# hongfz16/Garment4D

Hardware: AMD Instinct MI355X
Metric: point-cloud frames/s (FPS+ball_query+SA-MLP+LBS), B=8 N=8192 (higher is better)
Workload: dtype f32

## Files before the change

garment4d_amd/csrc/api.hip:

```cpp
#include <stdarg.h>
#include <stddef.h>
#include <stdlib.h>
#include <string.h>

#include "mlp_common.h"

namespace g4d {
static thread_local char g_err[512] = "";

void set_error(const char *fmt, ...) {
    va_list ap;
    va_start(ap, fmt);
    vsnprintf(g_err, sizeof(g_err), fmt, ap);
    va_end(ap);
}

static int g_contract = -1;

static int parse_contract(const char *e) {
    if (!e || !*e) return G4D_CONTRACT_NVCC;
    if (!strcmp(e, "0") || !strcmp(e, "off") || !strcmp(e, "none")) return G4D_CONTRACT_OFF;
    if (!strcmp(e, "2") || !strcmp(e, "chain") || !strcmp(e, "inner")) return G4D_CONTRACT_CHAIN;
    return G4D_CONTRACT_NVCC;
}

static thread_local int t_contract = -1;

int distance_contraction() {
    if (t_contract >= 0) return t_contract;
    int m = __atomic_load_n(&g_contract, __ATOMIC_RELAXED);
    if (m < 0) {
        m = parse_contract(getenv("G4D_DIST_CONTRACT"));
        __atomic_store_n(&g_contract, m, __ATOMIC_RELAXED);
    }
    return m;
}
}

namespace g4d {
namespace {
struct Tune { const char *key; long long value; int state; };
Tune g_tune[] = {{"sa_table_persistent", 0, 0}, {"sa_table_min_rows", 0, 0}, {"sa_table_128", 0, 0}, {"sa_table_oversub", 0, 0}, {"sa_table_dedup", 0, 0}, {"fp_table_persistent", 0, 0},
                 {"fp_table_min_rows", 0, 0}, {"gemm_tile", 0, 0}, {"gemm_tile_min_rows", 0, 0}, {"gemm_tile_min_cout", 0, 0}, {"gemm_tile_min_kpad", 0, 0}, {"fp_init_persistent", 0, 0}, {"fp_init_min_rows", 0, 0},
                 {"fp_head_bf16_persistent", 0, 0}, {"fp_head_bf16_min_rows", 0, 0}, {"sa_group_bf16_persistent", 0, 0}, {"sa_group_bf16_min_rows", 0, 0}};
}
struct ThreadTune { long long value; bool set; };
thread_local ThreadTune t_tune[sizeof(g_tune) / sizeof(g_tune[0])] = {};

long long tuning(const char *key, long long dflt) {
    int i = 0;
    for (Tune &t : g_tune) {
        const int slot = i++;
        if (strcmp(t.key, key)) continue;
        if (t_tune[slot].set) return t_tune[slot].value;
        int st = __atomic_load_n(&t.state, __ATOMIC_ACQUIRE);
        if (st == 0) {
            char env[64] = "G4D_";
            size_t n = 4;
            for (const char *c = key; *c && n + 1 < sizeof(env); ++c) env[n++] = (char)((*c >= 'a' && *c <= 'z') ? *c - 32 : *c);
            env[n] = 0;
            const char *e = getenv(env);
            const long long v = e && *e ? atoll(e) : dflt;
            int expect = 0;
            if (__atomic_compare_exchange_n(&t.state, &expect, 3, false, __ATOMIC_ACQ_REL, __ATOMIC_ACQUIRE)) {
                __atomic_store_n(&t.value, v, __ATOMIC_RELAXED);
                expect = 3;
                __atomic_compare_exchange_n(&t.state, &expect, 1, false, __ATOMIC_ACQ_REL, __ATOMIC_ACQUIRE);
                return v;
            }
            st = expect;
            if (st == 3) return v;
        }
        return __atomic_load_n(&t.value, __ATOMIC_RELAXED);
    }
    return dflt;
}
}

extern "C" int g4d_tuning_set(const char *key, long long value) {
    if (key)
        for (g4d::Tune &t : g4d::g_tune)
            if (!strcmp(t.key, key)) {
                __atomic_store_n(&t.value, value, __ATOMIC_RELAXED);
                __atomic_store_n(&t.state, 2, __ATOMIC_RELEASE);
                return G4D_OK;
            }
    g4d::set_error("g4d_tuning_set: unknown key '%s'", key ? key : "(null)");
    return G4D_EINVAL;
}

extern "C" int g4d_tuning_set_thread(const char *key, long long value, int set) {
    if (key) {
        int i = 0;
        for (g4d::Tune &t : g4d::g_tune) {
            const int slot = i++;
            if (!strcmp(t.key, key)) {
                g4d::t_tune[slot].value = value;
                g4d::t_tune[slot].set = set != 0;
                return G4D_OK;
            }
        }
    }
    g4d::set_error("g4d_tuning_set_thread: unknown key '%s'", key ? key : "(null)");
    return G4D_EINVAL;
}

extern "C" int g4d_version(void) { return 263;  }
extern "C" const char *g4d_last_error(void) { return g4d::g_err; }

extern "C" int g4d_get_distance_contraction(void) { return g4d::distance_contraction(); }
extern "C" int g4d_set_distance_contraction_thread(int mode) {
    const int prev = g4d::t_contract;
    if (mode < -1 || mode > G4D_CONTRACT_CHAIN) {
        g4d::set_error("g4d_set_distance_contraction_thread: mode %d is not -1 (no override) or one of G4D_CONTRACT_OFF/NVCC/CHAIN", mode);
        return -2;
    }
    g4d::t_contract = mode;
    return prev;
}

extern "C" int g4d_set_distance_contraction(int mode) {
    const int saved = g4d::t_contract;
    g4d::t_contract = -1;
    const int prev = g4d::distance_contraction();
    g4d::t_contract = saved;
    if (mode < G4D_CONTRACT_OFF || mode > G4D_CONTRACT_CHAIN) {
        g4d::set_error("g4d_set_distance_contraction: mode %d is not one of G4D_CONTRACT_OFF/NVCC/CHAIN", mode);
        return -1;
    }
    __atomic_store_n(&g4d::g_contract, mode, __ATOMIC_RELAXED);
    return prev;
}

namespace g4d {
struct CopySegs { float *dst[4]; const float *src[4]; long long n[4]; long long first_block[5]; };
__global__ void __launch_bounds__(256) copy_segments_kernel(const CopySegs c, int nseg) {
    int s = 0;
    while (s + 1 < nseg && (long long)blockIdx.x >= c.first_block[s + 1]) ++s;
    const long long i0 = ((long long)blockIdx.x - c.first_block[s]) * 1024 + threadIdx.x * 4;
    float *d = c.dst[s];
    const float *p = c.src[s];
    const long long n = c.n[s];
    if (i0 + 3 < n && ((reinterpret_cast<size_t>(d) | reinterpret_cast<size_t>(p)) & 15) == 0) {
        *reinterpret_cast<float4 *>(d + i0) = *reinterpret_cast<const float4 *>(p + i0);
    } else {
        for (int e = 0; e < 4; ++e)
            if (i0 + e < n) d[i0 + e] = p[i0 + e];
    }
}
}

extern "C" int g4d_copy_segments_f32(int nseg, float *const *dst, const float *const *src, const long long *nfloats, g4d_stream_t stream) {
    G4D_REQUIRE(nseg >= 0 && nseg <= 4 && (nseg == 0 || (dst && src && nfloats)), "g4d_copy_segments_f32: 0..4 segments");
    g4d::CopySegs c = {};
    long long blocks = 0;
    int k = 0;
    for (int i = 0; i < nseg; ++i) {
        G4D_REQUIRE(nfloats[i] >= 0 && (nfloats[i] == 0 || (dst[i] && src[i])), "g4d_copy_segments_f32: bad segment %d", i);
        if (nfloats[i] == 0) continue;
        c.dst[k] = dst[i]; c.src[k] = src[i]; c.n[k] = nfloats[i]; c.first_block[k] = blocks;
        blocks += (nfloats[i] + 1023) / 1024;
        ++k;
    }
    if (k == 0) return G4D_OK;
    c.first_block[k] = blocks;
    G4D_REQUIRE(blocks < (1ll << 31), "g4d_copy_segments_f32: too large");
    hipLaunchKernelGGL(g4d::copy_segments_kernel, dim3((unsigned)blocks), dim3(256), 0, reinterpret_cast<hipStream_t>(stream), c, k);
    return g4d::check_launch("g4d_copy_segments_f32");
}

namespace g4d {
static StackCall stack_call(const char *name, const g4d_mlp_args &a) {
    StackCall c = {};
    c.name = name; c.mode = a.mode; c.rows = a.rows;
    LinearArgs &in = c.in;
    in.K = a.K0; in.out = a.out; in.ldo = a.ldo; in.col0 = a.col0; in.pool = a.pool; in.S = a.S;
    in.X = a.X; in.ldx = a.ldx;
    in.xyz = a.xyz; in.new_xyz = a.new_xyz; in.feats = a.feats; in.idx = a.idx; in.N = a.N; in.P = a.P; in.C = a.C; in.use_xyz = a.use_xyz;
    in.known_feats = a.known_feats; in.skip = a.skip; in.dist2 = a.dist2; in.nn_idx = a.nn_idx; in.C2 = a.C2; in.C1 = a.C1; in.m = a.m; in.n = a.n;
    in.rowptr = a.rowptr; in.colidx = a.colidx; in.vals = a.vals; in.Vg = a.Vg;
    c.nlayers = a.nlayers; c.W = a.W; c.scale = a.scale; c.shift = a.shift; c.Kpad = a.Kpad; c.Cout = a.Cout; c.relu = a.relu;
    c.tap_layer = a.tap_layer; c.tap_out = a.tap_out; c.tap_ld = a.tap_ld; c.unknown_grid = a.unknown_grid;
    return c;
}

int stack_call_check(const StackCall &c, const StackRules &r) {
    const int S = c.in.S, pool = c.in.pool;
    G4D_REQUIRE(c.mode >= 0 && c.mode <= (r.csr ? LOAD_CSR : LOAD_INTERP), "%s: %s", c.name, r.bad_mode);
    if (r.max_layers) G4D_REQUIRE(c.nlayers >= 1 && c.nlayers <= r.max_layers, "%s: 1..%d layers", c.name, r.max_layers);
    G4D_REQUIRE(c.rows >= 0 && c.rows < r.max_rows && c.in.K > 0, "%s: bad sizes", c.name);
    if (c.rows == 0) return kEmptyLaunch;
    G4D_REQUIRE(has_layer_arrays(c), "%s: null pointer", c.name);
    if (!r.max_layers) G4D_REQUIRE(g4d_mlp_chain_supported(c.nlayers, c.Cout), "%s: unsupported layer widths (see g4d_mlp_chain_supported)", c.name);
    G4D_REQUIRE(pool >= 0 && pool <= 2, "%s: pool must be 0|1|2", c.name);
    if (pool) G4D_REQUIRE((S == 4 || S == 8 || S == 16 || S == 32 || S == 64) && c.rows % S == 0, "%s: pooling needs S in {4,8,16,32,64}", c.name);
    for (int l = 0; l < c.nlayers; ++l) {
        const void *const *Wl = c.W + (size_t)l * r.w_pieces;
        G4D_REQUIRE(Wl[0] && (r.w_pieces == 1 || (Wl[1] && Wl[2])) && c.scale[l] && c.shift[l] && c.Kpad[l] % r.kpad_multiple == 0 && c.Cout[l] > 0, "%s: bad layer %d", c.name, l);
    }
    G4D_REQUIRE(tap_layer_of(c) < c.nlayers - 1, "%s: tap must be a hidden layer", c.name);
    return G4D_OK;
}
}

extern "C" unsigned g4d_mlp_args_size(void) { return (unsigned)sizeof(g4d_mlp_args); }

extern "C" int g4d_mlp_run(int family, const g4d_mlp_args *args, g4d_stream_t stream) {
    using namespace g4d;
    G4D_REQUIRE(args, "g4d_mlp_run: null argument block");
    G4D_REQUIRE(args->version == G4D_MLP_ARGS_VERSION, "g4d_mlp_run: argument block version %u, this library speaks %d", args->version, G4D_MLP_ARGS_VERSION);
    G4D_REQUIRE(args->size >= 16 && args->size <= sizeof(g4d_mlp_args), "g4d_mlp_run: argument block of %u bytes, this library's is %u (a newer caller?)",
                args->size, (unsigned)sizeof(g4d_mlp_args));
    g4d_mlp_args a;
    memset(&a, 0, sizeof(a));
    memcpy(&a, args, args->size);
    if (args->size < offsetof(g4d_mlp_args, tap_layer) + sizeof(int)) a.tap_layer = -1;
    if (family != G4D_MLP_CHAIN_BF16) a.unknown_grid = nullptr;
    hipStream_t st = reinterpret_cast<hipStream_t>(stream);
    switch (family) {
        case G4D_MLP_STACK_F32: return mlp_stack_f32_run(stack_call("g4d_mlp_stack_f32", a), st);
        case G4D_MLP_STACK_BF16: return mlp_stack_bf16_run(stack_call("g4d_mlp_stack_bf16", a), st);
        case G4D_MLP_WAVE_F32: return mlp_wave_f32_run(stack_call("g4d_mlp_wave_f32", a), st);
        case G4D_MLP_CHAIN_F32: return mlp_chain_f32_run(stack_call("g4d_mlp_chain_f32", a), st);
        case G4D_MLP_CHAIN_BF16: return mlp_chain_bf16_run(stack_call("g4d_mlp_chain_bf16", a), st);
        case G4D_MLP_CHAIN_BF16X3: return mlp_chain_bf16x3_run(stack_call("g4d_mlp_chain_bf16x3", a), st);
    }
    set_error("g4d_mlp_run: unknown kernel family %d", family);
    return G4D_EINVAL;
}

#define G4D_MLP_LOADERS                                                                                                                       \
    int mode, long long rows, int K0,  const float *X, int ldx,                                                            \
     int N, int P, int S, int C, int use_xyz, const float *xyz, const float *new_xyz, const float *feats, const int *idx,        \
     int n, int m, int C2, int C1, const float *known_feats, const float *skip, const float *dist2, const int *nn_idx
#define G4D_MLP_LAYERS(WT)                                                                                                                    \
    int nlayers, const WT *const *W, const float *const *scale, const float *const *shift, const int *Kpad, const int *Cout, const int *relu, \
     int pool, float *out, int ldo, int col0
#define G4D_MLP_COMMON                                                                                                                        \
    mode, rows, K0, X, ldx, N, P, S, C, use_xyz, xyz, new_xyz, feats, idx, n, m, C2, C1, known_feats, skip, dist2, nn_idx, nlayers,         \
    reinterpret_cast<const void *const *>(W), scale, shift, Kpad, Cout, relu, pool, out, ldo, col0

static g4d_mlp_args pack_args(G4D_MLP_LOADERS, G4D_MLP_LAYERS(void), int tap_layer = -1, float *tap_out = nullptr, int tap_ld = 0) {
    g4d_mlp_args a;
    memset(&a, 0, sizeof(a));
    a.size = (unsigned)sizeof(a); a.version = G4D_MLP_ARGS_VERSION;
    a.mode = mode; a.rows = rows; a.K0 = K0; a.X = X; a.ldx = ldx;
    a.N = N; a.P = P; a.S = S; a.C = C; a.use_xyz = use_xyz; a.xyz = xyz; a.new_xyz = new_xyz; a.feats = feats; a.idx = idx;
    a.n = n; a.m = m; a.C2 = C2; a.C1 = C1; a.known_feats = known_feats; a.skip = skip; a.dist2 = dist2; a.nn_idx = nn_idx;
    a.nlayers = nlayers; a.W = W; a.scale = scale; a.shift = shift; a.Kpad = Kpad; a.Cout = Cout; a.relu = relu;
    a.pool = pool; a.out = out; a.ldo = ldo; a.col0 = col0; a.tap_layer = tap_layer; a.tap_out = tap_out; a.tap_ld = tap_ld;
    return a;
}

extern "C" int g4d_mlp_stack_f32(G4D_MLP_LOADERS,  int Vg, const int *rowptr, const int *colidx, const float *vals, G4D_MLP_LAYERS(float),
                                 int tap_layer, float *tap_out, int tap_ld, g4d_stream_t stream) {
    g4d_mlp_args a = pack_args(G4D_MLP_COMMON, tap_layer, tap_out, tap_ld);
    a.Vg = Vg; a.rowptr = rowptr; a.colidx = colidx; a.vals = vals;
    return g4d_mlp_run(G4D_MLP_STACK_F32, &a, stream);
}

extern "C" int g4d_mlp_stack_bf16(G4D_MLP_LOADERS,  int Vg, const int *rowptr, const int *colidx, const float *vals, G4D_MLP_LAYERS(unsigned short),
                                  int tap_layer, float *tap_out, int tap_ld, g4d_stream_t stream) {
    g4d_mlp_args a = pack_args(G4D_MLP_COMMON, tap_layer, tap_out, tap_ld);
    a.Vg = Vg; a.rowptr = rowptr; a.colidx = colidx; a.vals = vals;
    return g4d_mlp_run(G4D_MLP_STACK_BF16, &a, stream);
}

extern "C" int g4d_mlp_wave_f32(G4D_MLP_LOADERS,  int Vg, const int *rowptr, const int *colidx, const float *vals, G4D_MLP_LAYERS(float),
                                g4d_stream_t stream) {
    g4d_mlp_args a = pack_args(G4D_MLP_COMMON);
    a.Vg = Vg; a.rowptr = rowptr; a.colidx = colidx; a.vals = vals;
    return g4d_mlp_run(G4D_MLP_WAVE_F32, &a, stream);
}

extern "C" int g4d_mlp_chain_f32(G4D_MLP_LOADERS, G4D_MLP_LAYERS(float), int tap_layer, float *tap_out, int tap_ld, g4d_stream_t stream) {
    g4d_mlp_args a = pack_args(G4D_MLP_COMMON, tap_layer, tap_out, tap_ld);
    return g4d_mlp_run(G4D_MLP_CHAIN_F32, &a, stream);
}

extern "C" int g4d_mlp_chain_bf16(G4D_MLP_LOADERS, G4D_MLP_LAYERS(unsigned short), int tap_layer, float *tap_out, int tap_ld, g4d_stream_t stream) {
    g4d_mlp_args a = pack_args(G4D_MLP_COMMON, tap_layer, tap_out, tap_ld);
    return g4d_mlp_run(G4D_MLP_CHAIN_BF16, &a, stream);
}

extern "C" int g4d_mlp_chain_cells_bf16(G4D_MLP_LOADERS, G4D_MLP_LAYERS(unsigned short), int tap_layer, float *tap_out, int tap_ld, const void *unknown_grid,
                                        g4d_stream_t stream) {
    g4d_mlp_args a = pack_args(G4D_MLP_COMMON, tap_layer, tap_out, tap_ld);
    a.unknown_grid = unknown_grid;
    return g4d_mlp_run(G4D_MLP_CHAIN_BF16, &a, stream);
}

extern "C" int g4d_mlp_chain_bf16x3(G4D_MLP_LOADERS, G4D_MLP_LAYERS(unsigned short), int tap_layer, float *tap_out, int tap_ld, g4d_stream_t stream) {
    g4d_mlp_args a = pack_args(G4D_MLP_COMMON, tap_layer, tap_out, tap_ld);
    return g4d_mlp_run(G4D_MLP_CHAIN_BF16X3, &a, stream);
}
```

garment4d_amd/csrc/fp_table.hip:

```cpp
#include <cstdlib>

#include "mlp_common.h"

namespace g4d {

typedef float f32x4u __attribute__((ext_vector_type(4), aligned(4)));

struct FpTabArgs {
    int rows, n, m;
    const float *tab;
    const float *dist2;
    const int *nn_idx;
    const unsigned char *perm_rec;
    size_t perm_stride;
    const float *ps, *pf;
    const float *W2, *sc2, *sh2, *W3, *sc3, *sh3, *W4, *sc4, *sh4;
    int cout4, relu4;
    float *out;  int ldo;
    float *tap;  int tap_ld;
};

constexpr int kC1 = 128, kC2 = 64, kC3 = 32, kC4 = 16;
constexpr int kT1 = kC1 / 16, kT2 = kC2 / 16, kT3 = kC3 / 16;
template <bool PERM, int kD, bool HEAD = true>
__global__ void __launch_bounds__(256, kD <= 4 ? 3 : 2) fp_table_head_kernel(const FpTabArgs a) {
    static_assert(kT1 % kD == 0, "ring depth divides the k-steps of a tile");
    constexpr int NW2 = kC1 * kC2, NW3 = kC2 * kC3, NW4 = kC3 * kC4;
    __shared__ __attribute__((aligned(16))) float s_w2[NW2], s_w3[NW3], s_w4[NW4];
    __shared__ __attribute__((aligned(16))) float s_ps[kC1], s_pf[kC1], s_sc2[kC2], s_sh2[kC2], s_sc3[kC3], s_sh3[kC3], s_sc4[kC4], s_sh4[kC4];
    const int tid = threadIdx.x;
    for (int i = tid; i < NW2 / 4; i += 256) reinterpret_cast<f32x4 *>(s_w2)[i] = reinterpret_cast<const f32x4 *>(a.W2)[i];
    if constexpr (HEAD) {
        for (int i = tid; i < NW3 / 4; i += 256) reinterpret_cast<f32x4 *>(s_w3)[i] = reinterpret_cast<const f32x4 *>(a.W3)[i];
        for (int i = tid; i < NW4 / 4; i += 256) reinterpret_cast<f32x4 *>(s_w4)[i] = reinterpret_cast<const f32x4 *>(a.W4)[i];
    }
    if (tid < kC1) { s_ps[tid] = a.ps[tid]; s_pf[tid] = a.pf[tid]; }
    if (tid < kC2) { s_sc2[tid] = a.sc2[tid]; s_sh2[tid] = a.sh2[tid]; }
    if constexpr (HEAD) {
        if (tid < kC3) { s_sc3[tid] = a.sc3[tid]; s_sh3[tid] = a.sh3[tid]; }
        if (tid < kC4) { s_sc4[tid] = a.sc4[tid]; s_sh4[tid] = a.sh4[tid]; }
    }
    __syncthreads();

    const int lane = tid & 63, wave = __builtin_amdgcn_readfirstlane(tid >> 6);
    const int fi = lane & 15, fq = lane >> 4;
    const int ntile = (a.rows + 15) >> 4;
    const int nwaves = gridDim.x * 4, wg = blockIdx.x * 4 + wave;
    if (wg >= ntile) return;
    const int iters = (ntile - wg + nwaves - 1) / nwaves;
    auto tile_of = [&](int it) { return min(wg + it * nwaves, ntile - 1); };

    struct Raw { int i0, i1, i2; float d0, d1, d2; int orow; };
    auto load_raw = [&](int tile) {
        Raw r;
        const int row = min(tile * 16 + fi, a.rows - 1);
        const int *ix = a.nn_idx + (size_t)row * 3;
        const float *dd = a.dist2 + (size_t)row * 3;
        r.i0 = ix[0]; r.i1 = ix[1]; r.i2 = ix[2];
        r.d0 = dd[0]; r.d1 = dd[1]; r.d2 = dd[2];
        const int b0 = __builtin_amdgcn_readfirstlane((tile * 16) / a.n);
        const int b = b0 + (row >= (b0 + 1) * a.n ? 1 : 0);
        r.orow = row;
        if constexpr (PERM) r.orow = b * a.n + reinterpret_cast<const int *>(a.perm_rec + (size_t)b * a.perm_stride)[4 * (row - b * a.n) + 3];
        return r;
    };
    struct Ctx { float w0, w1, w2; unsigned k0, k1, k2; int orow; };
    auto make = [&](int tile, const Raw &r) {
        Ctx c;
        const float r0 = 1.0f / (__fsqrt_rn(r.d0) + 1e-8f), r1 = 1.0f / (__fsqrt_rn(r.d1) + 1e-8f), r2 = 1.0f / (__fsqrt_rn(r.d2) + 1e-8f);
        const float norm = (r0 + r1) + r2;
        c.w0 = r0 / norm; c.w1 = r1 / norm; c.w2 = r2 / norm;
        const int row = min(tile * 16 + fi, a.rows - 1);
        const int b0 = __builtin_amdgcn_readfirstlane((tile * 16) / a.n);
        const unsigned base = (unsigned)(b0 + (row >= (b0 + 1) * a.n ? 1 : 0)) * (unsigned)a.m;
        c.k0 = (base + (unsigned)r.i0) * kC1 + fq * 4; c.k1 = (base + (unsigned)r.i1) * kC1 + fq * 4; c.k2 = (base + (unsigned)r.i2) * kC1 + fq * 4;
        c.orow = r.orow;
        return c;
    };
    struct Item { f32x4 t0, t1, t2; };
    auto load_item = [&](const Ctx &c, int ks) {
        Item x;
        x.t0 = *reinterpret_cast<const f32x4u *>(a.tab + c.k0 + ks * 16);
        x.t1 = *reinterpret_cast<const f32x4u *>(a.tab + c.k1 + ks * 16);
        x.t2 = *reinterpret_cast<const f32x4u *>(a.tab + c.k2 + ks * 16);
        return x;
    };

    Raw rawn = load_raw(tile_of(0));
    Ctx cur = make(tile_of(0), rawn);
    rawn = load_raw(tile_of(1));
    Item ring[kD];
#pragma unroll
    for (int d = 0; d < kD; ++d) ring[d] = load_item(cur, d);
    for (int it = 0; it < iters; ++it) {
        const int tile = tile_of(it);
        const Ctx nxt = make(tile_of(it + 1), rawn);
        rawn = load_raw(tile_of(it + 2));
        f32x4 h2[kT2];
#pragma unroll
        for (int ct = 0; ct < kT2; ++ct) h2[ct] = (f32x4){0.f, 0.f, 0.f, 0.f};
#pragma unroll
        for (int ks = 0; ks < kT1; ++ks) {
            __builtin_amdgcn_sched_barrier(0);
            const Item x = ring[ks % kD];
            ring[ks % kD] = ks + kD < kT1 ? load_item(cur, ks + kD) : load_item(nxt, ks + kD - kT1);
            const int k0 = ks * 16 + fq * 4;
            const f32x4 ps = *reinterpret_cast<const f32x4 *>(s_ps + k0), pf = *reinterpret_cast<const f32x4 *>(s_pf + k0);
            f32x4 h1;
#pragma unroll
            for (int e = 0; e < 4; ++e) {
                const float v = cur.w0 * x.t0[e] + cur.w1 * x.t1[e] + cur.w2 * x.t2[e];
                h1[e] = fmaxf(__builtin_fmaf(v, ps[e], pf[e]), 0.f);
            }
#pragma unroll
            for (int ct = 0; ct < kT2; ++ct) {
                const f32x4 w = *reinterpret_cast<const f32x4 *>(s_w2 + ((ct * kT1 + ks) * 64 + lane) * 4);
#pragma unroll
                for (int e = 0; e < 4; ++e) h2[ct] = __builtin_amdgcn_mfma_f32_16x16x4f32(w[e], h1[e], h2[ct], 0, 0, 0);
            }
        }
        __builtin_amdgcn_sched_barrier(0);
        const bool row_ok = tile * 16 + fi < a.rows;
#pragma unroll
        for (int ct = 0; ct < kT2; ++ct) {
            const f32x4 sc = *reinterpret_cast<const f32x4 *>(s_sc2 + ct * 16 + fq * 4), sh = *reinterpret_cast<const f32x4 *>(s_sh2 + ct * 16 + fq * 4);
#pragma unroll
            for (int r = 0; r < 4; ++r) h2[ct][r] = fmaxf(__builtin_fmaf(h2[ct][r], sc[r], sh[r]), 0.f);
            if (row_ok) *reinterpret_cast<f32x4 *>(a.tap + (size_t)cur.orow * a.tap_ld + ct * 16 + fq * 4) = h2[ct];
        }
        if constexpr (HEAD) {
        __builtin_amdgcn_sched_barrier(0);
        f32x4 h3[kT3];
#pragma unroll
        for (int ct = 0; ct < kT3; ++ct) h3[ct] = (f32x4){0.f, 0.f, 0.f, 0.f};
#pragma unroll
        for (int ks = 0; ks < kT2; ++ks) {
            __builtin_amdgcn_sched_barrier(0);
#pragma unroll
            for (int ct = 0; ct < kT3; ++ct) {
                const f32x4 w = *reinterpret_cast<const f32x4 *>(s_w3 + ((ct * kT2 + ks) * 64 + lane) * 4);
#pragma unroll
                for (int e = 0; e < 4; ++e) h3[ct] = __builtin_amdgcn_mfma_f32_16x16x4f32(w[e], h2[ks][e], h3[ct], 0, 0, 0);
            }
        }
        __builtin_amdgcn_sched_barrier(0);
#pragma unroll
        for (int ct = 0; ct < kT3; ++ct) {
            const f32x4 sc = *reinterpret_cast<const f32x4 *>(s_sc3 + ct * 16 + fq * 4), sh = *reinterpret_cast<const f32x4 *>(s_sh3 + ct * 16 + fq * 4);
#pragma unroll
            for (int r = 0; r < 4; ++r) h3[ct][r] = fmaxf(__builtin_fmaf(h3[ct][r], sc[r], sh[r]), 0.f);
        }
        __builtin_amdgcn_sched_barrier(0);
        f32x4 o = (f32x4){0.f, 0.f, 0.f, 0.f};
#pragma unroll
        for (int ks = 0; ks < kT3; ++ks) {
            const f32x4 w = *reinterpret_cast<const f32x4 *>(s_w4 + (ks * 64 + lane) * 4);
#pragma unroll
            for (int e = 0; e < 4; ++e) o = __builtin_amdgcn_mfma_f32_16x16x4f32(h3[ks][e], w[e], o, 0, 0, 0);
        }
        {
            const float sc = s_sc4[fi], sh = s_sh4[fi];
#pragma unroll
            for (int r = 0; r < 4; ++r) {
                float y = __builtin_fmaf(o[r], sc, sh);
                if (a.relu4) y = fmaxf(y, 0.f);
                const int orow = __builtin_amdgcn_ds_bpermute((fq * 4 + r) << 2, cur.orow);
                if (fi < a.cout4 && tile * 16 + fq * 4 + r < a.rows) a.out[(size_t)orow * a.ldo + fi] = y;
            }
        }
        }
        cur = nxt;
    }
}

}

using namespace g4d;

int g4d::fp_table_try(const StackCall &c, hipStream_t st) {
    const LinearArgs &in = c.in;
    const float *const *W = reinterpret_cast<const float *const *>(c.W);
    float *tap_out = c.tap_out;
    int tap_ld = c.tap_ld;
    const int on = (int)tuning("fp_table_persistent", 1);
    const long long min_rows = tuning("fp_table_min_rows", 262144);
    const bool alone = c.nlayers == 1 && !tap_out && !in.in_tap && in.col0 == 0 && c.Cout[0] == kC2 && c.Kpad[0] == kC1 && c.relu[0];
    if (alone) { tap_out = in.out; tap_ld = in.ldo; }
    if (!on || c.rows < min_rows || c.rows >= (1ll << 31) - 64 || in.C2 != kC1 || (c.nlayers != 3 && !alone) || in.in_tap || in.col0 != 0 || (!alone && c.tap_layer != 0) || !tap_out) return -1;
    if (!alone && (c.Cout[0] != kC2 || c.Cout[1] != kC3 || c.Cout[2] > kC4 || c.Cout[2] < 1 || c.Kpad[0] != kC1 || c.Kpad[1] != kC2 || c.Kpad[2] != kC3 || !c.relu[0] || !c.relu[1])) return -1;
    if (in.n < 16 || in.m <= 0 || c.rows % in.n != 0 || (c.rows / in.n) * (long long)in.m * kC1 >= (1ll << 32) || tap_ld % 4 != 0 || (reinterpret_cast<size_t>(tap_out) & 15) != 0 ||
        (reinterpret_cast<size_t>(in.known_feats) & 15) != 0) return -1;
    G4D_REQUIRE(in.known_feats && in.dist2 && in.nn_idx && in.pre_scale && in.pre_shift && in.out && W[0] && c.scale[0] && c.shift[0] && (alone || (W[1] && W[2] && c.scale[1] && c.scale[2] && c.shift[1] && c.shift[2])),
                "g4d_mlp_chain_table_f32: null pointer");
    G4D_REQUIRE((alone || in.ldo >= c.Cout[2]) && tap_ld >= c.Cout[0], "g4d_mlp_chain_table_f32: output row stride %d or tap stride %d too small", in.ldo, tap_ld);
    FpTabArgs a;
    a.rows = (int)c.rows; a.n = in.n; a.m = in.m; a.tab = in.known_feats; a.dist2 = in.dist2; a.nn_idx = in.nn_idx;
    a.perm_rec = cell_records(c, &a.perm_stride);
    const unsigned char *perm_rec = a.perm_rec;
    a.ps = in.pre_scale; a.pf = in.pre_shift;
    a.W2 = W[0]; a.sc2 = c.scale[0]; a.sh2 = c.shift[0];
    a.W3 = alone ? nullptr : W[1]; a.sc3 = alone ? nullptr : c.scale[1]; a.sh3 = alone ? nullptr : c.shift[1];
    a.W4 = alone ? nullptr : W[2]; a.sc4 = alone ? nullptr : c.scale[2]; a.sh4 = alone ? nullptr : c.shift[2];
    a.cout4 = alone ? 0 : c.Cout[2]; a.relu4 = alone ? 0 : c.relu[2]; a.out = in.out; a.ldo = in.ldo; a.tap = tap_out; a.tap_ld = tap_ld;
    typedef void (*Kern)(const FpTabArgs);
    const Kern kern = alone ? (perm_rec ? fp_table_head_kernel<true, 2, false> : fp_table_head_kernel<false, 2, false>)
                            : (perm_rec ? fp_table_head_kernel<true, 2, true> : fp_table_head_kernel<false, 2, true>);
    static int resident[4] = {0, 0, 0, 0};
    int &res = resident[(perm_rec ? 1 : 0) + (alone ? 2 : 0)];
    if (res == 0) {
        int per_cu = 0, dev = 0;
        hipDeviceProp_t prop;
        if (hipOccupancyMaxActiveBlocksPerMultiprocessor(&per_cu, kern, 256, 0) != hipSuccess || per_cu < 1) per_cu = 1;
        res = (hipGetDevice(&dev) != hipSuccess || hipGetDeviceProperties(&prop, dev) != hipSuccess || prop.multiProcessorCount < 1) ? per_cu * 256 : per_cu * prop.multiProcessorCount;
    }
    const long long want = ((c.rows + 15) / 16 + 3) / 4;
    hipLaunchKernelGGL(kern, dim3((unsigned)(want < res ? want : res)), dim3(256), 0, st, a);
    return check_launch("g4d_fp_table_head");
}
```

garment4d_amd/tuning.py:

```python
import contextlib
import contextvars
import dataclasses
import os
from typing import Mapping, Tuple


def _env_flag(name, default):
    return os.environ.get(name, "1" if default else "0") != "0"


def _env_int(name, default):
    return int(os.environ.get(name, str(default)))


NATIVE_KEYS = ("sa_table_persistent", "sa_table_min_rows", "sa_table_128", "sa_table_oversub", "sa_table_dedup", "fp_table_persistent", "fp_table_min_rows", "gemm_tile",
               "gemm_tile_min_rows", "gemm_tile_min_cout", "gemm_tile_min_kpad", "fp_init_persistent", "fp_init_min_rows",
               "fp_head_bf16_persistent", "fp_head_bf16_min_rows", "sa_group_bf16_persistent", "sa_group_bf16_min_rows")


@dataclasses.dataclass(frozen=True)
class Tuning:
    use_wave: bool = True
    use_stack: bool = True
    use_chain: bool = True
    stream_gemm: bool = True
    bf16_min_rows: int = 0
    overlap_sampling: bool = False
    lanes_sort: bool = False
    coherent_lanes: bool = False
    grid_min_n: int = 4096
    fps_pair: bool = True
    bq_multi: bool = True
    search_multi: bool = True
    three_nn_grid_min_m: int = 4096
    nn_cells: bool = True
    nn_multi: bool = True
    nn_prune: bool = True
    sa_xyz_pair: bool = True
    use_sa_xyz: bool = True
    sa_xyz_table: bool = True
    sa_table: bool = True
    fp_wide_fused: bool = False
    fp_cells: bool = True
    fp_table: bool = True
    fp_gemm_bf16: bool = True
    fp_gemm_bf16_min_rows: int = 8192
    fp_wide_table: bool = True
    dropin_fused: bool = True
    dropin_whole_model: bool = True
    use_pe_kernel: bool = True
    gcn_fuse_stack: bool = True
    gcn_autograd: bool = False
    refine_autograd: bool = False
    mgn_autograd: bool = False
    stage1_autograd: bool = False
    mlp_autograd: bool = False
    lbs_fused: bool = True
    lbs_mfma: bool = True
    lbs_one_launch: bool = True
    lbs_one_launch_max_b: int = 1 << 30
    nearest_cull: bool = True
    native: Tuple[Tuple[str, int], ...] = ()

    def replace(self, **kw) -> "Tuning":
        nat = kw.pop("native", None)
        if nat is not None:
            if isinstance(nat, Mapping):
                merged = dict(self.native)
                merged.update({str(k): int(v) for k, v in nat.items()})
                nat = tuple(sorted(merged.items()))
            else:
                nat = tuple((str(k), int(v)) for k, v in nat)
            for k, _ in nat:
                if k not in NATIVE_KEYS:
                    raise KeyError(f"unknown native tuning key '{k}' (include/g4d.h lists them)")
            kw["native"] = nat
        return dataclasses.replace(self, **kw)


def from_environment() -> Tuning:
    d = Tuning()
    return Tuning(
        use_wave=_env_flag("G4D_MLP_WAVE", d.use_wave), use_chain=_env_flag("G4D_MLP_CHAIN", d.use_chain), stream_gemm=_env_flag("G4D_GEMM_STREAM", d.stream_gemm),
        bf16_min_rows=_env_int("G4D_BF16_MIN_ROWS", d.bf16_min_rows), overlap_sampling=_env_flag("G4D_OVERLAP_SAMPLING", d.overlap_sampling),
        lanes_sort=_env_flag("G4D_BQ_LANES_SORT", d.lanes_sort), coherent_lanes=_env_flag("G4D_BQ_LANES", d.coherent_lanes),
        grid_min_n=_env_int("G4D_BQ_GRID_MIN_N", d.grid_min_n), fps_pair=_env_flag("G4D_FPS_PAIR", d.fps_pair), bq_multi=_env_flag("G4D_BQ_MULTI", d.bq_multi),
        search_multi=_env_flag("G4D_SEARCH_MULTI", d.search_multi), three_nn_grid_min_m=_env_int("G4D_NN_GRID_MIN_M", d.three_nn_grid_min_m),
        nn_cells=_env_flag("G4D_NN_CELLS", d.nn_cells), nn_multi=_env_flag("G4D_NN_MULTI", d.nn_multi), nn_prune=_env_flag("G4D_NN_PRUNE", d.nn_prune), sa_xyz_pair=_env_flag("G4D_SA_XYZ_PAIR", d.sa_xyz_pair),
        use_sa_xyz=_env_flag("G4D_SA_XYZ", d.use_sa_xyz), sa_xyz_table=_env_flag("G4D_SA_XYZ_TABLE", d.sa_xyz_table), sa_table=_env_flag("G4D_SA_TABLE", d.sa_table),
        fp_wide_fused=_env_flag("G4D_FP_WIDE_FUSED", d.fp_wide_fused), fp_cells=_env_flag("G4D_FP_CELLS", d.fp_cells), fp_table=_env_flag("G4D_FP_TABLE", d.fp_table),
        fp_gemm_bf16=_env_flag("G4D_FP_GEMM_BF16", d.fp_gemm_bf16), fp_gemm_bf16_min_rows=_env_int("G4D_FP_GEMM_BF16_MIN_ROWS", d.fp_gemm_bf16_min_rows),
        fp_wide_table=_env_flag("G4D_FP_WIDE_TABLE", d.fp_wide_table), gcn_fuse_stack=_env_flag("G4D_GCN_FUSED", d.gcn_fuse_stack), gcn_autograd=_env_flag("G4D_GCN_AUTOGRAD", d.gcn_autograd),
        refine_autograd=_env_flag("G4D_REFINE_AUTOGRAD", d.refine_autograd), mgn_autograd=_env_flag("G4D_MGN_AUTOGRAD", d.mgn_autograd),
        stage1_autograd=_env_flag("G4D_STAGE1_AUTOGRAD", d.stage1_autograd), mlp_autograd=_env_flag("G4D_MLP_AUTOGRAD", d.mlp_autograd),
        dropin_fused=_env_flag("G4D_DROPIN_FUSED", d.dropin_fused), dropin_whole_model=_env_flag("G4D_DROPIN_WHOLE", d.dropin_whole_model), lbs_mfma=_env_flag("G4D_LBS_MFMA", d.lbs_mfma), lbs_one_launch=_env_flag("G4D_LBS_ONE", d.lbs_one_launch),
        lbs_one_launch_max_b=_env_int("G4D_LBS_ONE_MAX_B", d.lbs_one_launch_max_b), nearest_cull=_env_flag("G4D_NEAREST_CULL", d.nearest_cull))


DEFAULT = from_environment()
_CURRENT = contextvars.ContextVar("g4d_tuning", default=DEFAULT)


def current() -> Tuning:
    return _CURRENT.get()


@contextlib.contextmanager
def use(t: Tuning):
    outer = _CURRENT.get()
    token = _CURRENT.set(t)
    touched = {k for k, _ in t.native} | {k for k, _ in outer.native}
    try:
        if touched:
            _apply_native(dict(t.native), touched)
        yield t
    finally:
        _CURRENT.reset(token)
        if touched:
            _apply_native(dict(outer.native), touched)


def _apply_native(values, keys):
    from . import _lib
    for k in keys:
        if k in values:
            _lib.call("g4d_tuning_set_thread", k.encode(), int(values[k]), 1)
        else:
            _lib.call("g4d_tuning_set_thread", k.encode(), 0, 0)
```

Before: 51600.

## Process two row tiles per wave in FP table head kernel with weight-fragment ring

The fused feature-propagation table/MLP head kernel now has each wave handle two 16-row tiles per unit. Each weight fragment loaded from LDS feeds MFMAs for both tiles. Weight fragments are prefetched through a register ring, and per-row contexts are computed once and distributed with ds_bpermute. Next-unit index, weight and affine loads are staggered inside the k-loop, and a tuning knob caps the grid size. The changes aim to cut LDS weight traffic and hide gather latency, at the cost of more register pressure and fewer units, and so possibly less parallelism.

```diff
diff --git a/garment4d_amd/csrc/api.hip b/garment4d_amd/csrc/api.hip
--- a/garment4d_amd/csrc/api.hip
+++ b/garment4d_amd/csrc/api.hip
@@ -41,7 +41,7 @@
 namespace {
 struct Tune { const char *key; long long value; int state; };
 Tune g_tune[] = {{"sa_table_persistent", 0, 0}, {"sa_table_min_rows", 0, 0}, {"sa_table_128", 0, 0}, {"sa_table_oversub", 0, 0}, {"sa_table_dedup", 0, 0}, {"fp_table_persistent", 0, 0},
-                 {"fp_table_min_rows", 0, 0}, {"gemm_tile", 0, 0}, {"gemm_tile_min_rows", 0, 0}, {"gemm_tile_min_cout", 0, 0}, {"gemm_tile_min_kpad", 0, 0}, {"fp_init_persistent", 0, 0}, {"fp_init_min_rows", 0, 0},
+                 {"fp_table_min_rows", 0, 0}, {"fp_table_max_wgs", 0, 0}, {"gemm_tile", 0, 0}, {"gemm_tile_min_rows", 0, 0}, {"gemm_tile_min_cout", 0, 0}, {"gemm_tile_min_kpad", 0, 0}, {"fp_init_persistent", 0, 0}, {"fp_init_min_rows", 0, 0},
                  {"fp_head_bf16_persistent", 0, 0}, {"fp_head_bf16_min_rows", 0, 0}, {"sa_group_bf16_persistent", 0, 0}, {"sa_group_bf16_min_rows", 0, 0}};
 }
 struct ThreadTune { long long value; bool set; };
diff --git a/garment4d_amd/csrc/fp_table.hip b/garment4d_amd/csrc/fp_table.hip
--- a/garment4d_amd/csrc/fp_table.hip
+++ b/garment4d_amd/csrc/fp_table.hip
@@ -22,9 +22,13 @@
 
 constexpr int kC1 = 128, kC2 = 64, kC3 = 32, kC4 = 16;
 constexpr int kT1 = kC1 / 16, kT2 = kC2 / 16, kT3 = kC3 / 16;
+constexpr int kMT = 2;
+constexpr int kRD = 4;
+constexpr int kKD = 1;
 template <bool PERM, int kD, bool HEAD = true>
-__global__ void __launch_bounds__(256, kD <= 4 ? 3 : 2) fp_table_head_kernel(const FpTabArgs a) {
-    static_assert(kT1 % kD == 0, "ring depth divides the k-steps of a tile");
+__global__ void __launch_bounds__(256, 3) fp_table_head_kernel(const FpTabArgs a) {
+    static_assert(kT1 % kD == 0 && 2 * kD <= kT1, "ring depth divides the k-steps of a tile; the next contexts are staged in the k-steps in front of it");
+    constexpr int MT = kMT, RD = kRD;
     constexpr int NW2 = kC1 * kC2, NW3 = kC2 * kC3, NW4 = kC3 * kC4;
     __shared__ __attribute__((aligned(16))) float s_w2[NW2], s_w3[NW3], s_w4[NW4];
     __shared__ __attribute__((aligned(16))) float s_ps[kC1], s_pf[kC1], s_sc2[kC2], s_sh2[kC2], s_sc3[kC3], s_sh3[kC3], s_sc4[kC4], s_sh4[kC4];
@@ -44,132 +48,194 @@
 
     const int lane = tid & 63, wave = __builtin_amdgcn_readfirstlane(tid >> 6);
     const int fi = lane & 15, fq = lane >> 4;
-    const int ntile = (a.rows + 15) >> 4;
+    const int ntile = (a.rows + 15) >> 4, nunit = (ntile + MT - 1) / MT;
     const int nwaves = gridDim.x * 4, wg = blockIdx.x * 4 + wave;
-    if (wg >= ntile) return;
-    const int iters = (ntile - wg + nwaves - 1) / nwaves;
-    auto tile_of = [&](int it) { return min(wg + it * nwaves, ntile - 1); };
-
-    struct Raw { int i0, i1, i2; float d0, d1, d2; int orow; };
-    auto load_raw = [&](int tile) {
+    if (wg >= nunit) return;
+    const int iters = (nunit - wg + nwaves - 1) / nwaves;
+    auto unit_of = [&](int it) { return min(wg + it * nwaves, nunit - 1); };
+    const int lrow = lane & (16 * MT - 1);
+    struct Raw { int i0, i1, i2; float d0, d1, d2; int orow; unsigned base; };
+    auto load_raw = [&](int unit) {
         Raw r;
-        const int row = min(tile * 16 + fi, a.rows - 1);
+        const int row = min(unit * (16 * MT) + lrow, a.rows - 1);
         const int *ix = a.nn_idx + (size_t)row * 3;
         const float *dd = a.dist2 + (size_t)row * 3;
         r.i0 = ix[0]; r.i1 = ix[1]; r.i2 = ix[2];
         r.d0 = dd[0]; r.d1 = dd[1]; r.d2 = dd[2];
-        const int b0 = __builtin_amdgcn_readfirstlane((tile * 16) / a.n);
-        const int b = b0 + (row >= (b0 + 1) * a.n ? 1 : 0);
+        const int b0 = __builtin_amdgcn_readfirstlane((unit * (16 * MT)) / a.n);
+        const int b = b0 + (row >= (b0 + 1) * a.n ? 1 : 0) + (row >= (b0 + 2) * a.n ? 1 : 0);
+        r.base = (unsigned)b * (unsigned)a.m;
         r.orow = row;
         if constexpr (PERM) r.orow = b * a.n + reinterpret_cast<const int *>(a.perm_rec + (size_t)b * a.perm_stride)[4 * (row - b * a.n) + 3];
         return r;
     };
     struct Ctx { float w0, w1, w2; unsigned k0, k1, k2; int orow; };
-    auto make = [&](int tile, const Raw &r) {
+    auto make = [&](const Raw &r) {
         Ctx c;
         const float r0 = 1.0f / (__fsqrt_rn(r.d0) + 1e-8f), r1 = 1.0f / (__fsqrt_rn(r.d1) + 1e-8f), r2 = 1.0f / (__fsqrt_rn(r.d2) + 1e-8f);
         const float norm = (r0 + r1) + r2;
         c.w0 = r0 / norm; c.w1 = r1 / norm; c.w2 = r2 / norm;
-        const int row = min(tile * 16 + fi, a.rows - 1);
-        const int b0 = __builtin_amdgcn_readfirstlane((tile * 16) / a.n);
-        const unsigned base = (unsigned)(b0 + (row >= (b0 + 1) * a.n ? 1 : 0)) * (unsigned)a.m;
-        c.k0 = (base + (unsigned)r.i0) * kC1 + fq * 4; c.k1 = (base + (unsigned)r.i1) * kC1 + fq * 4; c.k2 = (base + (unsigned)r.i2) * kC1 + fq * 4;
+        c.k0 = (r.base + (unsigned)r.i0) * kC1; c.k1 = (r.base + (unsigned)r.i1) * kC1; c.k2 = (r.base + (unsigned)r.i2) * kC1;
         c.orow = r.orow;
         return c;
     };
+    auto take = [&](int v, int mt) { return __builtin_amdgcn_ds_bpermute((mt * 16 + fi) << 2, v); };
+    auto hand_k = [&](const Ctx &c, int mt, Ctx &t) { t.k0 = (unsigned)take((int)c.k0, mt); t.k1 = (unsigned)take((int)c.k1, mt); t.k2 = (unsigned)take((int)c.k2, mt); };
+    auto hand_w = [&](const Ctx &c, int mt, Ctx &t) {
+        t.w0 = __int_as_float(take(__float_as_int(c.w0), mt)); t.w1 = __int_as_float(take(__float_as_int(c.w1), mt)); t.w2 = __int_as_float(take(__float_as_int(c.w2), mt));
+    };
     struct Item { f32x4 t0, t1, t2; };
+    const float *tabq = a.tab + fq * 4;
     auto load_item = [&](const Ctx &c, int ks) {
         Item x;
-        x.t0 = *reinterpret_cast<const f32x4u *>(a.tab + c.k0 + ks * 16);
-        x.t1 = *reinterpret_cast<const f32x4u *>(a.tab + c.k1 + ks * 16);
-        x.t2 = *reinterpret_cast<const f32x4u *>(a.tab + c.k2 + ks * 16);
+        x.t0 = *reinterpret_cast<const f32x4u *>(tabq + c.k0 + ks * 16);
+        x.t1 = *reinterpret_cast<const f32x4u *>(tabq + c.k1 + ks * 16);
+        x.t2 = *reinterpret_cast<const f32x4u *>(tabq + c.k2 + ks * 16);
         return x;
     };
-
-    Raw rawn = load_raw(tile_of(0));
-    Ctx cur = make(tile_of(0), rawn);
-    rawn = load_raw(tile_of(1));
-    Item ring[kD];
-#pragma unroll
-    for (int d = 0; d < kD; ++d) ring[d] = load_item(cur, d);
+    constexpr int F2 = kT1 * kT2, F3 = HEAD ? kT2 * kT3 : 0, F = F2 + F3;
+    static_assert(F2 % RD == 0 && F % RD == 0 && RD <= F2, "the fragment ring keeps its slots across iterations");
+    auto wfrag = [&](int g) {
+        if (g < F2) return *reinterpret_cast<const f32x4 *>(s_w2 + (((g % kT2) * kT1 + g / kT2) * 64 + lane) * 4);
+        return *reinterpret_cast<const f32x4 *>(s_w3 + ((((g - F2) % kT3) * kT2 + (g - F2) / kT3) * 64 + lane) * 4);
+    };
+    auto aff_sc = [&](int j) { return *reinterpret_cast<const f32x4 *>((j < kT2 ? s_sc2 + j * 16 : s_sc3 + (j - kT2) * 16) + fq * 4); };
+    auto aff_sh = [&](int j) { return *reinterpret_cast<const f32x4 *>((j < kT2 ? s_sh2 + j * 16 : s_sh3 + (j - kT2) * 16) + fq * 4); };
+
+    Raw rawn = load_raw(unit_of(0));
+    Ctx made = make(rawn);
+    Ctx cur[MT], nxt[MT];
+#pragma unroll
+    for (int mt = 0; mt < MT; ++mt) { hand_k(made, mt, cur[mt]); hand_w(made, mt, cur[mt]); cur[mt].orow = take(made.orow, mt); }
+    Item tring[kD][MT];
+#pragma unroll
+    for (int d = 0; d < kD; ++d)
+#pragma unroll
+        for (int mt = 0; mt < MT; ++mt) tring[d][mt] = load_item(cur[mt], d);
+    f32x4 ring[RD];
+#pragma unroll
+    for (int f = 0; f < RD; ++f) ring[f] = wfrag(f);
+    f32x4 psn = *reinterpret_cast<const f32x4 *>(s_ps + fq * 4), pfn = *reinterpret_cast<const f32x4 *>(s_pf + fq * 4);
+    f32x4 scn, shn;
     for (int it = 0; it < iters; ++it) {
-        const int tile = tile_of(it);
-        const Ctx nxt = make(tile_of(it + 1), rawn);
-        rawn = load_raw(tile_of(it + 2));
-        f32x4 h2[kT2];
-#pragma unroll
-        for (int ct = 0; ct < kT2; ++ct) h2[ct] = (f32x4){0.f, 0.f, 0.f, 0.f};
+        const int unit = unit_of(it);
+        f32x4 h2[kT2][MT];
+#pragma unroll
+        for (int ct = 0; ct < kT2; ++ct)
+#pragma unroll
+            for (int mt = 0; mt < MT; ++mt) h2[ct][mt] = (f32x4){0.f, 0.f, 0.f, 0.f};
 #pragma unroll
         for (int ks = 0; ks < kT1; ++ks) {
+            f32x4 h1[MT];
+#pragma unroll
+            for (int mt = 0; mt < MT; ++mt) {
+                const Item x = tring[ks % kD][mt];
+#pragma unroll
+                for (int e = 0; e < 4; ++e) {
+                    const float v = cur[mt].w0 * x.t0[e] + cur[mt].w1 * x.t1[e] + cur[mt].w2 * x.t2[e];
+                    h1[mt][e] = fmaxf(__builtin_fmaf(v, psn[e], pfn[e]), 0.f);
+                }
+            }
+#pragma unroll
+            for (int ct = 0; ct < kT2; ++ct) {
+                const int g = ks * kT2 + ct;
+                const f32x4 w = ring[g % RD];
+                ring[g % RD] = wfrag((g + RD) % F);
+                __builtin_amdgcn_sched_barrier(0);
+                if (ct == 0) {
+                    const int kn = ((ks + 1) % kT1) * 16 + fq * 4;
+                    psn = *reinterpret_cast<const f32x4 *>(s_ps + kn); pfn = *reinterpret_cast<const f32x4 *>(s_pf + kn);
+#pragma unroll
+                    for (int mt = 0; mt < MT; ++mt)
+                        tring[ks % kD][mt] = ks + kD < kT1 ? load_item(cur[mt], ks + kD) : load_item(nxt[mt], ks + kD - kT1);
+                }
+                if (ks == 0 && ct == 1) rawn = load_raw(unit_of(it + 1));
+                if (ks == kT1 - kD - 1 && ct == 1) made = make(rawn);
+                if (ks == kT1 - kD - 1 && ct == 2) {
+#pragma unroll
+                    for (int mt = 0; mt < MT; ++mt) hand_k(made, mt, nxt[mt]);
+                }
+                if (ks == kT1 - 1 && ct == kT2 - 1) { scn = aff_sc(0); shn = aff_sh(0); }
+#pragma unroll
+                for (int e = 0; e < 4; ++e)
+#pragma unroll
+                    for (int mt = 0; mt < MT; ++mt) h2[ct][mt] = __builtin_amdgcn_mfma_f32_16x16x4f32(w[e], h1[mt][e], h2[ct][mt], 0, 0, 0);
+            }
+        }
+        bool row_ok[MT];
+#pragma unroll
+        for (int mt = 0; mt < MT; ++mt) { row_ok[mt] = (unit * MT + mt) * 16 + fi < a.rows; hand_w(made, mt, cur[mt]); }
+        auto finish2 = [&](int ct) {
+            const f32x4 sc = scn, sh = shn;
+            if (ct + 1 < kT2 + (HEAD ? kT3 : 0)) { scn = aff_sc(ct + 1); shn = aff_sh(ct + 1); }
+#pragma unroll
+            for (int mt = 0; mt < MT; ++mt) {
+#pragma unroll
+                for (int r = 0; r < 4; ++r) h2[ct][mt][r] = fmaxf(__builtin_fmaf(h2[ct][mt][r], sc[r], sh[r]), 0.f);
+                if (row_ok[mt]) *reinterpret_cast<f32x4 *>(a.tap + (size_t)cur[mt].orow * a.tap_ld + ct * 16 + fq * 4) = h2[ct][mt];
+            }
+        };
+        if constexpr (!HEAD) {
+#pragma unroll
+            for (int ct = 0; ct < kT2; ++ct) finish2(ct);
+        } else {
+        f32x4 h3[kT3][MT];
+#pragma unroll
+        for (int ct = 0; ct < kT3; ++ct)
+#pragma unroll
+            for (int mt = 0; mt < MT; ++mt) h3[ct][mt] = (f32x4){0.f, 0.f, 0.f, 0.f};
+        f32x4 w4[kT3];
+        float sc4 = 0.f, sh4 = 0.f;
+#pragma unroll
+        for (int ks = 0; ks < kT2; ++ks) {
+            finish2(ks);
+            if (ks == kT2 - 2) {
+#pragma unroll
+                for (int k4 = 0; k4 < kT3; ++k4) w4[k4] = *reinterpret_cast<const f32x4 *>(s_w4 + (k4 * 64 + lane) * 4);
+            }
+            if (ks == kT2 - 1) { sc4 = s_sc4[fi]; sh4 = s_sh4[fi]; }
+#pragma unroll
+            for (int ct = 0; ct < kT3; ++ct) {
+                const int g = F2 + ks * kT3 + ct;
+                const f32x4 w = ring[g % RD];
+                ring[g % RD] = wfrag((g + RD) % F);
+                __builtin_amdgcn_sched_barrier(0);
+#pragma unroll
+                for (int e = 0; e < 4; ++e)
+#pragma unroll
+                    for (int mt = 0; mt < MT; ++mt) h3[ct][mt] = __builtin_amdgcn_mfma_f32_16x16x4f32(w[e], h2[ks][mt][e], h3[ct][mt], 0, 0, 0);
+            }
+        }
+        f32x4 o[MT];
+#pragma unroll
+        for (int mt = 0; mt < MT; ++mt) o[mt] = (f32x4){0.f, 0.f, 0.f, 0.f};
+#pragma unroll
+        for (int ks = 0; ks < kT3; ++ks) {
+            const f32x4 sc = scn, sh = shn;
+            if (ks + 1 < kT3) { scn = aff_sc(kT2 + ks + 1); shn = aff_sh(kT2 + ks + 1); }
+#pragma unroll
+            for (int mt = 0; mt < MT; ++mt)
+#pragma unroll
+                for (int r = 0; r < 4; ++r) h3[ks][mt][r] = fmaxf(__builtin_fmaf(h3[ks][mt][r], sc[r], sh[r]), 0.f);
             __builtin_amdgcn_sched_barrier(0);
-            const Item x = ring[ks % kD];
-            ring[ks % kD] = ks + kD < kT1 ? load_item(cur, ks + kD) : load_item(nxt, ks + kD - kT1);
-            const int k0 = ks * 16 + fq * 4;
-            const f32x4 ps = *reinterpret_cast<const f32x4 *>(s_ps + k0), pf = *reinterpret_cast<const f32x4 *>(s_pf + k0);
-            f32x4 h1;
-#pragma unroll
-            for (int e = 0; e < 4; ++e) {
-                const float v = cur.w0 * x.t0[e] + cur.w1 * x.t1[e] + cur.w2 * x.t2[e];
-                h1[e] = fmaxf(__builtin_fmaf(v, ps[e], pf[e]), 0.f);
-            }
-#pragma unroll
-            for (int ct = 0; ct < kT2; ++ct) {
-                const f32x4 w = *reinterpret_cast<const f32x4 *>(s_w2 + ((ct * kT1 + ks) * 64 + lane) * 4);
-#pragma unroll
-                for (int e = 0; e < 4; ++e) h2[ct] = __builtin_amdgcn_mfma_f32_16x16x4f32(w[e], h1[e], h2[ct], 0, 0, 0);
-            }
+#pragma unroll
+            for (int e = 0; e < 4; ++e)
+#pragma unroll
+                for (int mt = 0; mt < MT; ++mt) o[mt] = __builtin_amdgcn_mfma_f32_16x16x4f32(h3[ks][mt][e], w4[ks][e], o[mt], 0, 0, 0);
         }
         __builtin_amdgcn_sched_barrier(0);
-        const bool row_ok = tile * 16 + fi < a.rows;
-#pragma unroll
-        for (int ct = 0; ct < kT2; ++ct) {
-            const f32x4 sc = *reinterpret_cast<const f32x4 *>(s_sc2 + ct * 16 + fq * 4), sh = *reinterpret_cast<const f32x4 *>(s_sh2 + ct * 16 + fq * 4);
-#pragma unroll
-            for (int r = 0; r < 4; ++r) h2[ct][r] = fmaxf(__builtin_fmaf(h2[ct][r], sc[r], sh[r]), 0.f);
-            if (row_ok) *reinterpret_cast<f32x4 *>(a.tap + (size_t)cur.orow * a.tap_ld + ct * 16 + fq * 4) = h2[ct];
-        }
-        if constexpr (HEAD) {
-        __builtin_amdgcn_sched_barrier(0);
-        f32x4 h3[kT3];
-#pragma unroll
-        for (int ct = 0; ct < kT3; ++ct) h3[ct] = (f32x4){0.f, 0.f, 0.f, 0.f};
-#pragma unroll
-        for (int ks = 0; ks < kT2; ++ks) {
-            __builtin_amdgcn_sched_barrier(0);
-#pragma unroll
-            for (int ct = 0; ct < kT3; ++ct) {
-                const f32x4 w = *reinterpret_cast<const f32x4 *>(s_w3 + ((ct * kT2 + ks) * 64 + lane) * 4);
-#pragma unroll
-                for (int e = 0; e < 4; ++e) h3[ct] = __builtin_amdgcn_mfma_f32_16x16x4f32(w[e], h2[ks][e], h3[ct], 0, 0, 0);
-            }
-        }
-        __builtin_amdgcn_sched_barrier(0);
-#pragma unroll
-        for (int ct = 0; ct < kT3; ++ct) {
-            const f32x4 sc = *reinterpret_cast<const f32x4 *>(s_sc3 + ct * 16 + fq * 4), sh = *reinterpret_cast<const f32x4 *>(s_sh3 + ct * 16 + fq * 4);
-#pragma unroll
-            for (int r = 0; r < 4; ++r) h3[ct][r] = fmaxf(__builtin_fmaf(h3[ct][r], sc[r], sh[r]), 0.f);
-        }
-        __builtin_amdgcn_sched_barrier(0);
-        f32x4 o = (f32x4){0.f, 0.f, 0.f, 0.f};
-#pragma unroll
-        for (int ks = 0; ks < kT3; ++ks) {
-            const f32x4 w = *reinterpret_cast<const f32x4 *>(s_w4 + (ks * 64 + lane) * 4);
-#pragma unroll
-            for (int e = 0; e < 4; ++e) o = __builtin_amdgcn_mfma_f32_16x16x4f32(h3[ks][e], w[e], o, 0, 0, 0);
-        }
-        {
-            const float sc = s_sc4[fi], sh = s_sh4[fi];
+#pragma unroll
+        for (int mt = 0; mt < MT; ++mt)
 #pragma unroll
             for (int r = 0; r < 4; ++r) {
-                float y = __builtin_fmaf(o[r], sc, sh);
+                float y = __builtin_fmaf(o[mt][r], sc4, sh4);
                 if (a.relu4) y = fmaxf(y, 0.f);
-                const int orow = __builtin_amdgcn_ds_bpermute((fq * 4 + r) << 2, cur.orow);
-                if (fi < a.cout4 && tile * 16 + fq * 4 + r < a.rows) a.out[(size_t)orow * a.ldo + fi] = y;
-            }
-        }
-        }
-        cur = nxt;
+                const int orow = __builtin_amdgcn_ds_bpermute((fq * 4 + r) << 2, cur[mt].orow);
+                if (fi < a.cout4 && (unit * MT + mt) * 16 + fq * 4 + r < a.rows) a.out[(size_t)orow * a.ldo + fi] = y;
+            }
+        }
+#pragma unroll
+        for (int mt = 0; mt < MT; ++mt) { cur[mt].k0 = nxt[mt].k0; cur[mt].k1 = nxt[mt].k1; cur[mt].k2 = nxt[mt].k2; cur[mt].orow = take(made.orow, mt); }
     }
 }
 
@@ -203,8 +269,8 @@
     a.W4 = alone ? nullptr : W[2]; a.sc4 = alone ? nullptr : c.scale[2]; a.sh4 = alone ? nullptr : c.shift[2];
     a.cout4 = alone ? 0 : c.Cout[2]; a.relu4 = alone ? 0 : c.relu[2]; a.out = in.out; a.ldo = in.ldo; a.tap = tap_out; a.tap_ld = tap_ld;
     typedef void (*Kern)(const FpTabArgs);
-    const Kern kern = alone ? (perm_rec ? fp_table_head_kernel<true, 2, false> : fp_table_head_kernel<false, 2, false>)
-                            : (perm_rec ? fp_table_head_kernel<true, 2, true> : fp_table_head_kernel<false, 2, true>);
+    const Kern kern = alone ? (perm_rec ? fp_table_head_kernel<true, kKD, false> : fp_table_head_kernel<false, kKD, false>)
+                            : (perm_rec ? fp_table_head_kernel<true, kKD, true> : fp_table_head_kernel<false, kKD, true>);
     static int resident[4] = {0, 0, 0, 0};
     int &res = resident[(perm_rec ? 1 : 0) + (alone ? 2 : 0)];
     if (res == 0) {
@@ -213,7 +279,10 @@
         if (hipOccupancyMaxActiveBlocksPerMultiprocessor(&per_cu, kern, 256, 0) != hipSuccess || per_cu < 1) per_cu = 1;
         res = (hipGetDevice(&dev) != hipSuccess || hipGetDeviceProperties(&prop, dev) != hipSuccess || prop.multiProcessorCount < 1) ? per_cu * 256 : per_cu * prop.multiProcessorCount;
     }
-    const long long want = ((c.rows + 15) / 16 + 3) / 4;
-    hipLaunchKernelGGL(kern, dim3((unsigned)(want < res ? want : res)), dim3(256), 0, st, a);
+    const long long want = (((c.rows + 15) / 16 + kMT - 1) / kMT + 3) / 4;
+    const long long max_wgs = tuning("fp_table_max_wgs", 0);
+    long long grid = want < res ? want : res;
+    if (max_wgs > 0 && grid > max_wgs) grid = max_wgs;
+    hipLaunchKernelGGL(kern, dim3((unsigned)grid), dim3(256), 0, st, a);
     return check_launch("g4d_fp_table_head");
 }
diff --git a/garment4d_amd/tuning.py b/garment4d_amd/tuning.py
--- a/garment4d_amd/tuning.py
+++ b/garment4d_amd/tuning.py
@@ -13,7 +13,7 @@
     return int(os.environ.get(name, str(default)))
 
 
-NATIVE_KEYS = ("sa_table_persistent", "sa_table_min_rows", "sa_table_128", "sa_table_oversub", "sa_table_dedup", "fp_table_persistent", "fp_table_min_rows", "gemm_tile",
+NATIVE_KEYS = ("sa_table_persistent", "sa_table_min_rows", "sa_table_128", "sa_table_oversub", "sa_table_dedup", "fp_table_persistent", "fp_table_min_rows", "fp_table_max_wgs", "gemm_tile",
                "gemm_tile_min_rows", "gemm_tile_min_cout", "gemm_tile_min_kpad", "fp_init_persistent", "fp_init_min_rows",
                "fp_head_bf16_persistent", "fp_head_bf16_min_rows", "sa_group_bf16_persistent", "sa_group_bf16_min_rows")
 
```

After: 52200 (median of 6 runs). 1.01x the previous value.
